# ishine/ASR-Rescoring

Measured on AMD Instinct MI355X. Metric: masked-token BERT forwards/sec (MLM_PLL, N=50, L~32), higher is better.
Workload: dtype fp16x3-split (fp32-accurate: hi/lo fp16 operand split on fp16 MFMA, fp32 accumulate)

## Files before the change

### asr-rescoring_amd/_lib.py

```python
from __future__ import annotations

import ctypes
import os

import numpy as np
import torch

PKG_DIR = os.path.dirname(os.path.abspath(__file__))
LIB_PATH = os.environ.get("RS_LIBRESCORE") or os.path.join(PKG_DIR, "librescore.so")

RS_HEAD_MLM, RS_HEAD_CLS, RS_HEAD_EMB = 1, 2, 4
RS_FUSE = {"norm": 0, "legacy": 1, "am_norm": 2}
KINDS = ["qkv", "oproj", "ffn1", "ffn2", "decoder", "attn", "other"]


class RsBertCfg(ctypes.Structure):
    _fields_ = [("vocab", ctypes.c_int32), ("hidden", ctypes.c_int32), ("layers", ctypes.c_int32),
                ("heads", ctypes.c_int32), ("intermediate", ctypes.c_int32),
                ("max_pos", ctypes.c_int32), ("type_vocab", ctypes.c_int32),
                ("ln_eps", ctypes.c_float), ("mask_id", ctypes.c_int32),
                ("heads_mask", ctypes.c_int32), ("precision", ctypes.c_int32)]


RS_PREC = {"fp16": 0, "fp16x3": 1}
# ... 73 lines not shown
    "rs_trainer_destroy": (None, [P]),
    "rs_bertscore_recall": (ctypes.c_int, [P, P, P, P, I32, P, P, P]),
    "rs_align": (ctypes.c_int, [P, P, P, P, I32, P, P, P, P, P, P, P, I32, P]),
    "rs_fuse_rerank": (ctypes.c_int, [P, P, P, P, I32, I32, P, I32, I32, P, P]),
    "rs_corpus_edits": (ctypes.c_int, [P, P, P, I32, I32, P, P]),
    "rs_ref_edit": (ctypes.c_int, [P, P, P, P, P, I32, P, P]),
    "rs_vocab_load": (P, [ctypes.c_char_p]),
    "rs_vocab_size": (ctypes.c_int, [P]),
    "rs_vocab_free": (None, [P]),
    "rs_vocab_continuation": (ctypes.c_int, [P, P, I64, P]),
    "rs_tokenize_batch": (I64, [P, ctypes.POINTER(ctypes.c_char_p), I32, I32, P, I64, P]),
    "rs_json_write_scores": (ctypes.c_int, [ctypes.c_char_p, I32, ctypes.POINTER(ctypes.c_char_p), P,
                                            ctypes.POINTER(ctypes.c_char_p), P]),
}

CI = ctypes.c_int
_DEBUG_SIGS = {
    "rs_debug_gemm": (CI, [CI, CI, P, P, P, P, CI, CI, CI, P]),
    "rs_debug_attention": (CI, [CI, P, P, P, CI, CI, CI, P, P]),
    "rs_debug_ln": (CI, [CI, CI] + [P] * 9),
    "rs_debug_stamps": (CI, [CI, P]),
    "rs_debug_occupy": (CI, [CI, CI, P, P]),
    "rs_debug_sgemm_cfg": (CI, [CI] * 4 + [P, CI, CI, P, CI, CI, P, CI, CI, P]),
    "rs_debug_sgemm": (CI, [CI] * 3 + [P, CI, CI, P, CI, CI, P, CI, CI, P]),
    "rs_debug_sgemm_pick": (CI, [CI] * 5),
    "rs_debug_gelu": (CI, [P, P, CI, P]),
    "rs_debug_x3s": (CI, [CI, P, P, P, P, P, ctypes.c_float, P, CI, CI, CI, CI, CI, P, P, P, P]),
    "rs_debug_lnres_sizes": (CI, [CI, CI, ctypes.POINTER(I64)]),
    "rs_debug_attention_full": (CI, [P, P, P, CI, CI, CI, CI, CI, P, P]),
    "rs_debug_gemm_epi": (CI, [CI, P, P, CI, CI, CI, P, P]),
    "rs_debug_decoder": (CI, [P, P, P, P, CI, CI, CI, CI, CI, P, P, P, P, P]),
    "rs_debug_decoder_topk": (CI, [P, P, P, P, CI, CI, CI, CI, CI, P, P, P, P, CI, P, P, P, P]),
    "rs_debug_attention_query": (CI, [P, CI, P, P, P, CI, CI, CI, CI, CI, CI, P, P, P, P, P, P, P, P, P]),
    "rs_debug_train_attn": (CI, [CI, P, P, P, CI, CI, CI, P, ctypes.c_uint32, ctypes.c_uint64, ctypes.c_uint32,
                                 ctypes.c_float, P, P, P]),
    "rs_debug_train_embed_ln": (CI, [P, P, P, CI, CI, CI, CI, P, P, P, P, P, ctypes.c_float, CI, ctypes.c_uint32,
                                     ctypes.c_uint64, ctypes.c_uint32, ctypes.c_float, P, P, P, P]),
    "rs_debug_train_bias_res_ln": (CI, [P, P, P, CI, P, P, ctypes.c_float, CI, ctypes.c_uint32, ctypes.c_uint64,
                                        ctypes.c_uint32, ctypes.c_float, P, P, P]),
    "rs_debug_train_ln_bwd": (CI, [P, P, P, P, P, CI, CI, P]),
    "rs_debug_train_pointwise": (CI, [CI, P, P, P, CI, CI, P]),
    "rs_debug_train_colsum": (CI, [CI, P, P, P, CI, CI, P, P, CI, P, CI, P]),
    "rs_debug_train_word_grad": (CI, [P, P, P, P, CI, CI, CI, CI, P, P]),
    "rs_debug_train_pos_grad": (CI, [P, P, CI, CI, CI, CI, P, P]),
    "rs_debug_train_cls_fwd": (CI, [P, P, CI, CI, CI, P, P, P, P]),
    "rs_debug_train_cls_bwd": (CI, [P, P, P, CI, CI, CI, P, P, P, P, P]),
    "rs_debug_train_loss": (CI, [P, P, P, P, P, CI, CI, CI, ctypes.c_float, P, P, P, P]),
    "rs_debug_train_ce": (CI, [P, P, CI, CI, P, P, P]),
    "rs_debug_train_move_rows": (CI, [CI, P, P, CI, CI, CI, P, P]),
    "rs_debug_train_adamw": (CI, [P, P, P, P, I64] + [ctypes.c_float] * 5 + [I64, P]),
    "rs_debug_train_adamw_scaled": (CI, [P, P, P, P, I64] + [ctypes.c_float] * 6 + [I64, P]),
    "rs_debug_train_accum": (CI, [P, P, P, P, CI, I64, ctypes.c_float, P]),
    "rs_debug_train_sumsq": (CI, [P, P, P, CI, I64, P, P]),
    "rs_debug_bertscore_recall": (CI, [P, CI, CI, P, P, CI, P, P, P]),
    "rs_debug_embed_out": (CI, [P, P, P, P, P, P, P, P, CI, CI, CI, CI, CI, P, P]),
    "rs_debug_plan_unique": (CI, [P, P, P, P, CI, CI, CI, P, P]),
    "rs_debug_embed": (CI, [CI, P, P, P, CI, CI, CI, CI, CI, CI, CI, P, P, P, P, P, ctypes.c_float, CI, P, P, P, CI, P]),
    "rs_debug_attention_plan": (CI, [P, CI, P, CI, CI, CI, CI, CI, CI, CI, CI, P, P]),
    "rs_debug_attention_mquery": (CI, [P, CI, P, CI, CI, CI, CI, CI, P, P, P, P, P, P, P, P, P]),
    "rs_debug_gather": (CI, [CI, P, CI, P, P, CI, CI, CI, P, P, P, P]),
    "rs_debug_cls_linear": (CI, [P, CI, CI, P, P, P, P]),
    "rs_debug_segsum": (CI, [P, P, CI, P, P]),
}


class DebugGemmEpi(ctypes.Structure):
# ... 65 lines not shown
```

### asr-rescoring_amd/csrc/common.h

```cpp
#pragma once
#include <hip/hip_runtime.h>
#include <stdint.h>

typedef _Float16 f16;
typedef _Float16 half8 __attribute__((ext_vector_type(8)));
typedef _Float16 half4 __attribute__((ext_vector_type(4)));
typedef float f32x16 __attribute__((ext_vector_type(16)));
typedef float f32x4 __attribute__((ext_vector_type(4)));

#define RS_WAVE 64

enum EpiKind {
    EPI_BIAS_F16 = 0,
    EPI_GELU_F16 = 1,
    EPI_GELU_F32 = 2,
    EPI_RES_F32 = 3,
    EPI_LSE = 4,
    EPI_BIAS_F32 = 5,
    EPI_RESLN_F32 = 6,
    EPI_LNRES_IMG = 7,
    EPI_LSE_TOPK = 8,
};

struct EpiArgs {
// ... 125 lines not shown
}

hipError_t launch_embed_ln(const int* tok, const int* type, SeqMeta sm, int s0, int s1, int row0, int mask_id,
                           int vocab, int type_vocab, const float* word, const float* pos, const float* typetab,
                           const float* g, const float* b, float eps, int H, float* x32,
                           float2* stats, f16* h16, int kx, hipStream_t st);
hipError_t launch_ln_rows(const float* x, int rows, const float* g, const float* b, float eps,
                          int H, float* y32, float2* stats, f16* y16, int kx, hipStream_t st);
hipError_t launch_ln_res_rows(float* x32, const float2* stats, float2* stats_out, const float* pg, const float* pb,
                             const f16* o16, int rows, const float* g, const float* b, float eps, int H,
                             f16* y16, bool write_x, hipStream_t st, const float2* stats1 = nullptr,
                             const float* g1 = nullptr, const float* b1 = nullptr, const f16* o16b = nullptr);
hipError_t launch_ln_res32(float* x32, const float2* stats, float2* stats_out, const float* pg, const float* pb,
                           const float* o32, int rows, const float* g, const float* b, float eps, int H, f16* y16,
                           int kx, hipStream_t st);
hipError_t launch_ln_res_img(f16* h16, const float* o32, int rows, const float* g, const float* b, float eps, int H,
                             hipStream_t st);
hipError_t launch_embed_unique(const int* tok, const int* type, SeqMeta sm, int s0, int s1, int urows, int mask_id,
                               int vocab, int type_vocab, const float* word, const float* pos, const float* typetab,
                               const float* g, const float* b, float eps, int H, f16* h16u, int kx, hipStream_t st);
int bertscore_cols(bool two);
hipError_t launch_bertscore_recall(const f16* emb, int H, const int* hyp_off, const int* utt_off,
                                   const long long* mat_off, const int4* items, int n_items, float* rmat, float* rmat0,
                                   hipStream_t st, bool two = false);
hipError_t launch_embed_out(const float* x32, const float2* stats, const float* g, const float* b,
                            SeqMeta sm, int s0, int s1, int row0, int H, f16* out, hipStream_t st,
                            const f16* himg = nullptr, bool two = false);
hipError_t launch_attention_full(const void* qkv, bool qkv32, SeqMeta sm, int s0, int s1, int row0,
                                 int H, int heads, f16* ctx, int kx, hipStream_t st, bool dedup, int max_len);
hipError_t launch_attention_query(const void* qkv, bool qkv32, const float* x32, const float2* stats,
                                  const float* g, const float* b, SeqMeta sm, int s0, int s1,
                                  int row0, int H, int heads, f16* ctxq, float* resq, int kx,
                                  hipStream_t st, const void* qd = nullptr, const f16* himg = nullptr);
hipError_t launch_gather_query_rows(const f16* src, int ld, SeqMeta sm, int s0, int s1, int row0, f16* dst,
                                   hipStream_t st);
hipError_t launch_gather_labels(const int* tok, SeqMeta sm, int s0, int s1, int* lab, float* label_logit,
                                hipStream_t st);
hipError_t launch_lse_finalize(const float2* part, int n_parts, const float* label_logit,
                               int rows, float* out, hipStream_t st);
hipError_t launch_embed_ln_set(const int* tok, const int* type, SeqMeta sm, QueryMeta qm, int s0, int s1, int mask_id,
                               int vocab, int type_vocab, const float* word, const float* pos, const float* typetab,
                               const float* g, const float* b, float eps, int H, float* x32, float2* stats, f16* h16,
                               int kx, hipStream_t st);
hipError_t launch_attention_mquery(const void* qkv, bool qkv32, const float* x32, const float2* stats, const float* g,
                                   const float* b, SeqMeta sm, QueryMeta qm, int s0, int s1, int H, int heads,
                                   f16* ctxq, float* resq, int kx, hipStream_t st, const void* qd = nullptr,
                                   const f16* himg = nullptr);
hipError_t launch_gather_query_rows_list(const f16* src, int ld, SeqMeta sm, QueryMeta qm, int q0, int n, f16* dst,
                                        hipStream_t st);
hipError_t launch_gather_labels_list(const int* tok, SeqMeta sm, QueryMeta qm, int q0, int n, int* lab,
                                     float* label_logit, hipStream_t st);

struct MlmDecoder {
    const f16* A;
    const f16* W;
    const float* bias;
    int m_valid, vpad, vocab, K;
    const int* tok;
    SeqMeta sm;
    int s0;
    int* lab;
    float2* part;
    float* llog;
    float* out;
    const QueryMeta* qm = nullptr;
};
// ... 52 lines not shown
```

### asr-rescoring_amd/csrc/k_attn.hip

```cpp
#include <type_traits>
#include "common.h"

namespace {

typedef __fp16 fp16x4 __attribute__((__vector_size__(4 * sizeof(__fp16))));

__device__ __forceinline__ half4 tr_read(const f16* p) {
    const fp16x4 v = __builtin_amdgcn_ds_read_tr16_b64_v4f16((__attribute__((address_space(3))) fp16x4*)p);
    return __builtin_bit_cast(half4, v);
}

template <class QT, bool DEDUP>
struct SeqRows {
    const QT* base;
    const QT* mbase;
    int ld, lo, n;
    __device__ __forceinline__ SeqRows(const QT* qkv, const SeqMeta& sm, int s, int rs, int ld_, int hd) : ld(ld_) {
        const int ub = DEDUP ? sm.urow_h[s] : rs;
        lo = DEDUP ? sm.mask_pos[s] : 0;
        n = DEDUP ? sm.mask_end[s] - lo : 0;
        const int um = DEDUP ? sm.urow_m[s] - lo : 0;
        base = qkv + (size_t)ub * ld + hd * 64;
        mbase = qkv + (ptrdiff_t)um * ld + hd * 64;
    }
// ... 582 lines not shown
                float d = 0.f;
#pragma unroll
                for (int c = 0; c < 8; ++c) {
                    float kv[8];
                    load8(kr + c * 8, kv);
#pragma unroll
                    for (int e = 0; e < 8; ++e) d += sq[w][c * 8 + e] * kv[e];
                }
                sc = d;
            }
            const float mn = fmaxf(m, wave_max(sc));
            const float p = (j < T) ? __expf(sc - mn) : 0.f;
            const float alpha = __expf(m - mn);
            l = l * alpha + wave_sum(p);
            acc *= alpha;
            __syncthreads();
            sp[w][lane] = p;
            __syncthreads();
            const int nk = min(64, T - k0);
            for (int jj = 0; jj < nk; ++jj)
                acc += sp[w][jj] * (float)base[(size_t)(k0 + jj) * ld + 2 * H + lane];
            m = mn;
        }
        if (on) {
            put_split(ctxq + (size_t)q_loc * kx * H, h * 64 + lane, H, kx, acc / l);
            const int c = h * 64 + lane;
            const size_t r = (size_t)(rs + qi);
            const float2 hl = himg ? il_parts(himg + r * 2 * H, c) : make_float2(0.f, 0.f);
            resq[(size_t)q_loc * H + c] = himg ? hl.x + hl.y * X3_DOWN : ln_apply(x32[r * H + c], stats[r], lg[c], lb[c]);
        }
    }
}

__global__ void __launch_bounds__(256)
attn_memskel_kernel(const f16* __restrict__ qkv, SeqMeta sm, int H, f16* __restrict__ ctx, int heads_per_block) {
    const int s = blockIdx.x;
    const int T = sm.len[s], rs = sm.row[s];
    const int lane = threadIdx.x & 63, hd = blockIdx.y * heads_per_block + (threadIdx.x >> 6);
    const int ld = 3 * H;
    const f16* base = qkv + (size_t)rs * ld + hd * 64;
    for (int r0 = 0; r0 < T; r0 += 8) {
        const int t = r0 + (lane >> 3), d0 = (lane & 7) * 8;
        if (t < T) {
            const half8 q = *(const half8*)(base + (size_t)t * ld + d0);
            const half8 k = *(const half8*)(base + (size_t)t * ld + H + d0);
            const half8 v = *(const half8*)(base + (size_t)t * ld + 2 * H + d0);
            *(half8*)(ctx + (size_t)(rs + t) * H + hd * 64 + d0) = q + k + v;
        }
    }
}

enum AttnKind {
    ATTN_TR = 0,
    ATTN_MEMSKEL_1 = 3,
    ATTN_MEMSKEL_4 = 4,
    ATTN_16 = 6,
    ATTN_FULL_F32 = 9,
    ATTN_X3_48 = 10,
    ATTN_X3_64 = 11,
};

}

hipError_t launch_attention_full(const void* qkv, bool qkv32, SeqMeta sm, int s0, int s1, int row0,
                                 int H, int heads, f16* ctx, int kx, hipStream_t st, bool dedup, int max_len) {
    if (s1 <= s0) return hipSuccess;
// ... 12 lines not shown
            if (max_len <= 64) hipLaunchKernelGGL(attn16_kernel<D>, grid, block, 0, st, q, sm, s0, row0, H, ctx, kx);
            else hipLaunchKernelGGL(attn_tr_kernel<D>, grid, block, 0, st, q, sm, s0, row0, H, ctx, kx);
        }
    };
    if (dedup) route(std::true_type{});
    else route(std::false_type{});
    return hipGetLastError();
}

hipError_t launch_attention_query(const void* qkv, bool qkv32, const float* x32, const float2* stats,
                                  const float* g, const float* b, SeqMeta sm, int s0, int s1,
                                  int row0, int H, int heads, f16* ctxq, float* resq, int kx,
                                  hipStream_t st, const void* qd, const f16* himg) {
    if (s1 <= s0) return hipSuccess;
    const dim3 grid(s1 - s0, heads);
    if (qkv32)
        hipLaunchKernelGGL(attn_query_kernel<float>, grid, dim3(64), 0, st, (const float*)qkv, (const float*)qd, x32, stats, g, b, sm, s0, row0, H, ctxq, resq, kx, himg);
    else
        hipLaunchKernelGGL(attn_query_kernel<f16>, grid, dim3(64), 0, st, (const f16*)qkv, (const f16*)qd, x32, stats, g, b, sm, s0, row0, H, ctxq, resq, kx, himg);
    return hipGetLastError();
}

hipError_t launch_attention_mquery(const void* qkv, bool qkv32, const float* x32, const float2* stats, const float* g,
                                   const float* b, SeqMeta sm, QueryMeta qm, int s0, int s1, int H, int heads,
                                   f16* ctxq, float* resq, int kx, hipStream_t st, const void* qd, const f16* himg) {
    if (s1 <= s0) return hipSuccess;
    if (H != heads * 64) return hipErrorInvalidValue;
    const dim3 grid(s1 - s0, heads);
    if (qkv32)
        hipLaunchKernelGGL(attn_mquery_kernel<float>, grid, dim3(256), 0, st, (const float*)qkv, (const float*)qd, x32, stats, g, b, sm, qm, s0, H, ctxq, resq, kx, himg);
    else
        hipLaunchKernelGGL(attn_mquery_kernel<f16>, grid, dim3(256), 0, st, (const f16*)qkv, (const f16*)qd, x32, stats, g, b, sm, qm, s0, H, ctxq, resq, kx, himg);
    return hipGetLastError();
}

extern "C" int rs_debug_attention(int kind, const void* qkv, const int* len, const int* row, int n_seq,
                                  int H, int heads, void* ctx, void* stream) {
    SeqMeta sm{};
    sm.len = len;
    sm.row = row;
    const dim3 grid(n_seq, heads), block(64);
    hipStream_t st = (hipStream_t)stream;
    const f16* q16 = (const f16*)qkv;
    const float* q32 = (const float*)qkv;
    f16* c = (f16*)ctx;
    switch (kind) {
        case ATTN_TR: hipLaunchKernelGGL(attn_tr_kernel<false>, grid, block, 0, st, q16, sm, 0, 0, H, c, 1); break;
        case ATTN_16: hipLaunchKernelGGL(attn16_kernel<false>, grid, block, 0, st, q16, sm, 0, 0, H, c, 1); break;
        case ATTN_FULL_F32: hipLaunchKernelGGL(attn_full_kernel<float>, grid, block, 0, st, q32, sm, 0, 0, H, c, 3, 0); break;
        case ATTN_X3_48: hipLaunchKernelGGL((attn16x3v2_kernel<false, 48>), grid, block, 0, st, q32, sm, 0, 0, H, c, 3); break;
        case ATTN_X3_64: hipLaunchKernelGGL((attn16x3v2_kernel<false, 64>), grid, block, 0, st, q32, sm, 0, 0, H, c, 3); break;
        case ATTN_MEMSKEL_1: hipLaunchKernelGGL(attn_memskel_kernel, grid, block, 0, st, q16, sm, H, c, 1); break;
        case ATTN_MEMSKEL_4:
            hipLaunchKernelGGL(attn_memskel_kernel, dim3(n_seq, heads / 4), dim3(256), 0, st, q16, sm, H, c, 4);
            break;
        default: return -1;
    }
    return hipGetLastError() == hipSuccess ? 0 : -2;
}

extern "C" int rs_debug_attention_full(const void* qkv32, const int* len, const int* row, int n_seq, int max_len,
                                       int H, int heads, int kx, void* ctx, void* stream) {
    if (!qkv32 || !len || !row || !ctx || n_seq <= 0 || max_len <= 0 || heads <= 0 || H != heads * 64) return -1;
    if (kx != 2 && kx != 3) return -1;
    SeqMeta sm{};
    sm.len = len;
// ... 46 lines not shown
```

### asr-rescoring_amd/csrc/rs_api.hip

```cpp
#include <map>
#include <string>
#include <vector>
#include <cstring>
#include <cstdio>
#include <cmath>
#include <algorithm>

#include "common.h"
#include "seq_plan.h"
#include "bertscore_plan.h"
#include "host_util.h"

namespace {

thread_local std::string g_err;

int fail(int code, const std::string& msg) {
    g_err = msg;
    return code;
}

struct Layer {
    f16 *wqkv, *wo, *w1, *w2;
    f16 *iqkv = nullptr, *io = nullptr, *i1 = nullptr, *i2 = nullptr;
    float *bqkv, *bo, *b1, *b2, *g1, *be1, *g2, *be2;
};

struct Staging {
    int* p = nullptr;
    size_t cap = 0;
    hipEvent_t done = nullptr;
    hipError_t begin(size_t n) {
        hipError_t e = done ? hipEventSynchronize(done) : hipSuccess;
        if (e == hipSuccess && n > cap) {
            if (p) (void)hipHostFree(p);
            p = nullptr;
            e = hipHostMalloc((void**)&p, std::max<size_t>(n, 1) * 4, hipHostMallocDefault);
            cap = e == hipSuccess ? n : 0;
        }
        return e;
    }
    hipError_t upload(DevBuf& dst, size_t n, hipStream_t st) {
        hipError_t e = dst.ensure(std::max<size_t>(n, 1) * 4);
        if (e == hipSuccess) e = hipMemcpyAsync(dst.p, p, n * 4, hipMemcpyHostToDevice, st);
        if (e == hipSuccess && !done) e = hipEventCreateWithFlags(&done, hipEventDisableTiming);
        return e == hipSuccess ? hipEventRecord(done, st) : e;
    }
    ~Staging() {
        if (p) (void)hipHostFree(p);
        if (done) (void)hipEventDestroy(done);
    }
};

}

struct rs_model {
    rs_bert_cfg cfg{};
    int device = 0;
// ... 270 lines not shown
    ~ProfScope() {
        if (m->prof && a) {
            hipEvent_t b = next_event(m);
            if (b) {
                (void)hipEventRecord(b, st);
                m->recs.push_back({kind, a, b, flops});
            }
        }
    }
};

#define LAUNCH(kind_, call_) do { ProfScope ps_(m, st, (kind_), 0); TRY_HIP(call_); } while (0)
#define LAUNCH_OTHER(call_) LAUNCH(RS_K_OTHER, call_)

enum Mode { MODE_MLM = 0, MODE_CLS = 1, MODE_EMB = 2 };

struct Call {
    int mode;
    const int* d_tok;
    float* out_rows = nullptr;
    const int* d_label = nullptr;
    const int32_t* d_type = nullptr;
    const std::vector<int>* extra = nullptr;
    int** d_extra = nullptr;
    f16* emb_dst = nullptr;
    int topk_k = 0;
    int32_t* topk_id = nullptr;
    float* topk_lp = nullptr;
    const QueryList* ql = nullptr;
};

struct CallOpts {
    bool lastq, dedup, chunk_align;
    int ln_diag;
    bool x3s, imgres, lnfuse, x3_dedup;
    bool oproj_f16, ffn2_f16;
    int lnres_defer;
};

CallOpts call_opts(const rs_model* m) {
    const rs_bert_cfg& cf = m->cfg;
    auto is = [](const char* name, const char* v) { const char* e = getenv(name); return e && !strcmp(e, v); };
    auto num = [](const char* name, int dflt) { const char* e = getenv(name); return e ? atoi(e) : dflt; };
    CallOpts o{};
    o.lastq = !is("RS_LASTQ", "0");
    o.dedup = num("RS_DEDUP", 1) != 0;
    o.chunk_align = !is("RS_CHUNK_ALIGN", "0");
    o.oproj_f16 = m->kx == 1 && !is("RS_OPROJ", "resln");
    o.ffn2_f16 = m->kx == 1 && is("RS_FFN2", "f16");
    const int defer = num("RS_LNRES_DEFER", 2);
    o.lnres_defer = !o.oproj_f16 || o.ffn2_f16 || defer == 0 ? 0 : defer == 2 ? 2 : 1;
    o.ln_diag = num("RS_LNFUSE_DIAG", 0) & 8;
    o.x3s = m->kx == 3 && !is("RS_X3S", "0") && m->x3s_w && cf.hidden % 256 == 0 && cf.intermediate % 256 == 0;
    o.imgres = o.x3s && !is("RS_X3S_IMGRES", "0");
    o.lnfuse = o.imgres && !is("RS_LNFUSE", "0") && cf.hidden % 256 == 0 && cf.hidden <= 1024;
    o.x3_dedup = o.imgres;
    return o;
}

struct ChunkCtx {
    rs_model* m;
    hipStream_t st;
    const Call& call;
    const SeqMeta& sm;
    const Chunk& c;
    const CallOpts& o;
    const QueryMeta& qm;
    const rs_bert_cfg& cf = m->cfg;
    const int H = cf.hidden, F = cf.intermediate, nh = cf.heads, kx = m->kx;
    const float eps = cf.ln_eps;
    const bool q32 = kx == 3;
    const int qkv_epi = q32 ? EPI_BIAS_F32 : EPI_BIAS_F16;
    const int rows = c.rows, ns = c.s1 - c.s0;
    const bool mq = call.ql != nullptr;
    const int nr = mq ? c.nq : ns, r0 = mq ? c.q0 : c.s0;
    const bool dedup = c.urows > 0;
    const int kxf = o.x3s ? 2 : kx;
    float2 *xst = m->xst.as<float2>(), *xst1 = m->xst1.as<float2>();
    float* t32 = m->t32.as<float>();
    f16* h16 = m->h16.as<f16>();
    void* qkv = m->qkv.p;
    f16 *ctx = m->ctx.as<f16>(), *inter = m->inter.as<f16>();
    f16 *ctxq = m->ctxq.as<f16>(), *hq16 = m->hq16.as<f16>(), *interq = m->interq.as<f16>();
    float *resq = m->resq.as<float>(), *tq = m->tq32.as<float>(), *hq32 = m->hq32.as<float>();

    int gemm(int kind, int epi, bool split, const f16* A, const f16* W, int m_valid, int N_pad, int K, EpiArgs ep,
             int n_flop_cols) {
        ep.m_valid = m_valid;
        ProfScope ps(m, st, kind, 2.0 * m_valid * (double)n_flop_cols * (split ? 3.0 * K : K));
// ... 15 lines not shown
    EpiArgs resln_ep(const float* bias, const float* lg, const float* lb) const {
        EpiArgs e = bias_ep(bias, t32, H, t32);
        e.res_stats = xst; e.res_g = lg; e.res_b = lb;
        return e;
    }
    const float* prev_g(int li) const { return li ? m->layers[li - 1].g2 : m->eg; }
    const float* prev_b(int li) const { return li ? m->layers[li - 1].be2 : m->eb; }
    int embed() {
        ProfScope ps(m, st, RS_K_OTHER, 0);
        if (mq && call.ql->masked) {
            TRY_HIP(launch_embed_ln_set(call.d_tok, call.d_type, sm, qm, c.s0, c.s1, cf.mask_id, cf.vocab, cf.type_vocab,
                                       m->word32, m->pos32, m->type32, m->eg, m->eb, eps, H, o.imgres ? nullptr : t32,
                                       o.imgres ? nullptr : xst, h16, kxf, st));
            return RS_OK;
        }
        TRY_HIP(launch_embed_ln(call.d_tok, call.d_type, sm, c.s0, c.s1, 0, cf.mask_id, cf.vocab, cf.type_vocab, m->word32,
                               m->pos32, m->type32, m->eg, m->eb, eps, H, o.imgres ? nullptr : t32,
                               o.imgres ? nullptr : xst, dedup && !o.x3s ? nullptr : h16, kxf, st));
        if (dedup)
            TRY_HIP(launch_embed_unique(call.d_tok, call.d_type, sm, c.s0, c.s1, c.urows, cf.mask_id, cf.vocab,
                                       cf.type_vocab, m->word32, m->pos32, m->type32, m->eg, m->eb, eps, H,
                                       o.x3s ? inter : h16, kxf, st));
        return RS_OK;
    }

    int qkv_proj(int li, bool last, bool uq, bool qrow) {
        const Layer& L = m->layers[li];
        const bool sp = o.x3s;
        const f16* W = sp ? L.iqkv : L.wqkv;
        const int K = sp ? H : kx * H, ldw = sp ? 2 * H : kx * H;
        if (!qrow)
            return gemm(RS_K_QKV, qkv_epi, sp, uq && sp ? inter : h16, W, uq ? c.urows : rows, 3 * H, K,
                        bias_ep(L.bqkv, qkv, 3 * H), last ? 2 * H : 3 * H);
        if (int r = gemm(RS_K_QKV, qkv_epi, sp, h16, W + (size_t)H * ldw, rows, 2 * H, K,
                         bias_ep(L.bqkv + H, (char*)qkv + H * (size_t)(q32 ? 4 : 2), 3 * H), 2 * H)) return r;
        if (mq) LAUNCH_OTHER(launch_gather_query_rows_list(h16, kxf * H, sm, qm, c.q0, c.nq, hq16, st));
        else LAUNCH_OTHER(launch_gather_query_rows(h16, kxf * H, sm, c.s0, c.s1, 0, hq16, st));
        return gemm(RS_K_QKV, qkv_epi, sp, hq16, W, nr, H, K, bias_ep(L.bqkv, tq, H), H);
    }

    int split_block(int kind, const f16* A, const f16* W, int K, const float* bias, const float* pg, const float* pb,
                    const float* g, const float* be) {
        if (o.lnfuse) {
            EpiArgs e = bias_ep(bias, h16, 2 * H);
            e.nlog = H; e.res_g = g; e.res_b = be; e.ln_eps = eps; e.lnx = m->lnx.p;
            e.lncnt = m->lncnt.as<unsigned>(); e.lnerr = m->lnerr.as<unsigned>(); e.diag = o.ln_diag;
            return gemm(kind, EPI_LNRES_IMG, true, A, W, rows, H, K, e, H);
        }
        float* o32 = (float*)qkv;
        if (int r = gemm(kind, EPI_BIAS_F32, true, A, W, rows, H, K, bias_ep(bias, o32, H), H)) return r;
        if (o.imgres) LAUNCH_OTHER(launch_ln_res_img(h16, o32, rows, g, be, eps, H, st));
        else LAUNCH_OTHER(launch_ln_res32(t32, xst, xst, pg, pb, o32, rows, g, be, eps, H, h16, 2, st));
        return RS_OK;
    }
    int layer_split(int li, bool uq) {
        const Layer& L = m->layers[li];
        LAUNCH(RS_K_ATTN, launch_attention_full(qkv, true, sm, c.s0, c.s1, 0, H, nh, ctx, 2, st, uq, c.max_len));
        if (int r = split_block(RS_K_OPROJ, ctx, L.io, H, L.bo, prev_g(li), prev_b(li), L.g1, L.be1)) return r;
        if (int r = gemm(RS_K_FFN1, EPI_GELU_F16, true, h16, L.i1, rows, F, H, gelu_ep(L.b1, inter, 2), F)) return r;
        return split_block(RS_K_FFN2, inter, L.i2, F, L.b2, L.g1, L.be1, L.g2, L.be2);
    }

    int layer_f16(int li, bool uq) {
        const Layer& L = m->layers[li];
        const float *pg = prev_g(li), *pb = prev_b(li);
        LAUNCH(RS_K_ATTN, launch_attention_full(qkv, q32, sm, c.s0, c.s1, 0, H, nh, ctx, kx, st, uq, c.max_len));
        f16* o16 = o.lnres_defer ? (f16*)qkv : inter;
        if (!o.oproj_f16) {
            if (int r = gemm(RS_K_OPROJ, EPI_RESLN_F32, false, ctx, L.wo, rows, H, kx * H, resln_ep(L.bo, pg, pb), H))
                return r;
            LAUNCH_OTHER(launch_ln_rows(t32, rows, L.g1, L.be1, eps, H, nullptr, xst, h16, kx, st));
        } else {
            if (int r = gemm(RS_K_OPROJ, EPI_BIAS_F16, false, ctx, L.wo, rows, H, H, bias_ep(L.bo, o16, H), H)) return r;
            if (o.lnres_defer)
                LAUNCH_OTHER(launch_ln_res_rows(t32, xst, xst1, pg, pb, o16, rows, L.g1, L.be1, eps, H, h16, false, st));
            else
                LAUNCH_OTHER(launch_ln_res_rows(t32, xst, xst, pg, pb, o16, rows, L.g1, L.be1, eps, H, h16, true, st));
        }
        if (int r = gemm(RS_K_FFN1, EPI_GELU_F16, false, h16, L.w1, rows, F, kx * H, gelu_ep(L.b1, inter, kx), F)) return r;
        if (o.lnres_defer == 2) {
            if (int r = gemm(RS_K_FFN2, EPI_BIAS_F16, false, inter, L.w2, rows, H, F, bias_ep(L.b2, ctx, H), H)) return r;
            LAUNCH_OTHER(launch_ln_res_rows(t32, xst, xst, pg, pb, o16, rows, L.g2, L.be2, eps, H, h16, true, st, xst1,
                                            L.g1, L.be1, ctx));
        } else if (o.ffn2_f16) {
            if (int r = gemm(RS_K_FFN2, EPI_BIAS_F16, false, inter, L.w2, rows, H, F, bias_ep(L.b2, ctx, H), H)) return r;
            LAUNCH_OTHER(launch_ln_res_rows(t32, xst, xst, L.g1, L.be1, ctx, rows, L.g2, L.be2, eps, H, h16, true, st));
        } else if (o.lnres_defer == 1) {
            EpiArgs ep = resln_ep(L.b2, L.g1, L.be1);
            ep.res_stats = xst1; ep.res_o16 = o16; ep.res_stats0 = xst; ep.res_g0 = pg; ep.res_b0 = pb;
            if (int r = gemm(RS_K_FFN2, EPI_RESLN_F32, false, inter, L.w2, rows, H, kx * F, ep, H)) return r;
            LAUNCH_OTHER(launch_ln_rows(t32, rows, L.g2, L.be2, eps, H, nullptr, xst, h16, kx, st));
        } else {
            if (int r = gemm(RS_K_FFN2, EPI_RESLN_F32, false, inter, L.w2, rows, H, kx * F, resln_ep(L.b2, L.g1, L.be1), H))
                return r;
            LAUNCH_OTHER(launch_ln_rows(t32, rows, L.g2, L.be2, eps, H, nullptr, xst, h16, kx, st));
        }
        return RS_OK;
    }

    int layer_query(int li, bool qrow) {
        const Layer& L = m->layers[li];
        if (mq)
            LAUNCH(RS_K_ATTN, launch_attention_mquery(qkv, q32, t32, xst, prev_g(li), prev_b(li), sm, qm, c.s0, c.s1, H, nh,
                                                      ctxq, resq, kx, st, qrow ? tq : nullptr, o.imgres ? h16 : nullptr));
        else
            LAUNCH(RS_K_ATTN, launch_attention_query(qkv, q32, t32, xst, prev_g(li), prev_b(li), sm, c.s0, c.s1, 0, H, nh,
                                                     ctxq, resq, kx, st, qrow ? tq : nullptr, o.imgres ? h16 : nullptr));
        if (int r = gemm(RS_K_OPROJ, EPI_RES_F32, false, ctxq, L.wo, nr, H, kx * H, bias_ep(L.bo, tq, H, resq), H))
            return r;
        LAUNCH_OTHER(launch_ln_rows(tq, nr, L.g1, L.be1, eps, H, hq32, nullptr, hq16, kx, st));
        if (int r = gemm(RS_K_FFN1, EPI_GELU_F16, false, hq16, L.w1, nr, F, kx * H, gelu_ep(L.b1, interq, kx), F)) return r;
        if (int r = gemm(RS_K_FFN2, EPI_RES_F32, false, interq, L.w2, nr, H, kx * F, bias_ep(L.b2, tq, H, hq32), H))
            return r;
        LAUNCH_OTHER(launch_ln_rows(tq, nr, L.g2, L.be2, eps, H, hq32, nullptr, hq16, kx, st));
        return RS_OK;
    }

    int head_mlm() {
        if (int r = gemm(RS_K_DECODER, EPI_GELU_F32, false, hq16, m->wt, nr, H, kx * H, bias_ep(m->bt, tq, H), H)) return r;
        LAUNCH_OTHER(launch_ln_rows(tq, nr, m->gt, m->bet, eps, H, hq32, nullptr, hq16, kx, st));
        const MlmDecoder d{hq16, m->wdec, m->bdec, nr, m->vpad, cf.vocab, kx * H, call.d_tok, sm, r0, m->lab.as<int>(),
                           m->part.as<float2>(), m->llog.as<float>(), call.out_rows + r0, mq ? &qm : nullptr};
        if (call.topk_k) {
            const int k = call.topk_k, n_gemm = (ns + TOPK_SUB_ROWS - 1) / TOPK_SUB_ROWS;
            const MlmTopk t{k, m->topk_cand.as<float2>(), call.topk_id + (size_t)c.s0 * k, call.topk_lp + (size_t)c.s0 * k};
            TRY_HIP(launch_mlm_decoder_topk(d, t, st, [&](bool is_gemm, auto&& launch) {
                ProfScope ps(m, st, is_gemm ? RS_K_DECODER : RS_K_OTHER,
                             is_gemm ? 2.0 * ns * (double)cf.vocab * (kx * H) / n_gemm : 0);
                return launch();
            }));
            return RS_OK;
        }
        TRY_HIP(launch_mlm_decoder(d, st, [&](bool is_gemm, auto&& launch) {
            ProfScope ps(m, st, is_gemm ? RS_K_DECODER : RS_K_OTHER, is_gemm ? 2.0 * nr * (double)cf.vocab * (kx * H) : 0);
            return launch();
// ... 333 lines not shown
        auto* bq = need(m, p + "attention.self.query.bias", H, &miss);
        auto* wk = need(m, p + "attention.self.key.weight", H * H, &miss);
        auto* bk = need(m, p + "attention.self.key.bias", H, &miss);
        auto* wv = need(m, p + "attention.self.value.weight", H * H, &miss);
        auto* bv = need(m, p + "attention.self.value.bias", H, &miss);
        auto* wo = need(m, p + "attention.output.dense.weight", H * H, &miss);
        auto* bo = need(m, p + "attention.output.dense.bias", H, &miss);
        auto* g1 = need(m, p + "attention.output.LayerNorm.weight", H, &miss);
        auto* be1 = need(m, p + "attention.output.LayerNorm.bias", H, &miss);
        auto* w1 = need(m, p + "intermediate.dense.weight", F * H, &miss);
        auto* b1 = need(m, p + "intermediate.dense.bias", F, &miss);
        auto* w2 = need(m, p + "output.dense.weight", H * F, &miss);
        auto* b2 = need(m, p + "output.dense.bias", H, &miss);
        auto* g2 = need(m, p + "output.LayerNorm.weight", H, &miss);
        auto* be2 = need(m, p + "output.LayerNorm.bias", H, &miss);
        if (!miss.empty()) return fail(RS_ESTATE, "tensor " + miss);
        std::vector<float> wqkv, bqkv;
        wqkv.reserve(3 * H * H);
        for (auto* w : {wq, wk, wv}) wqkv.insert(wqkv.end(), w->begin(), w->end());
        for (auto* b : {bq, bk, bv}) bqkv.insert(bqkv.end(), b->begin(), b->end());
        Layer& L = m->layers[i];
        UP16(L.wqkv, &wqkv, 3 * H, H);
        UP32(L.bqkv, &bqkv, 3 * H);
        UP16(L.wo, wo, H, H);
        UP32(L.bo, bo, H);
        UP32(L.g1, g1, H);
        UP32(L.be1, be1, H);
        UP16(L.w1, w1, F, H);
        UP32(L.b1, b1, F);
        UP16(L.w2, w2, H, F);
        UP32(L.b2, b2, H);
        UP32(L.g2, g2, H);
        UP32(L.be2, be2, H);
        if (x3s_w) {
            UPIL(L.iqkv, &wqkv, H);
            UPIL(L.io, wo, H);
            UPIL(L.i1, w1, H);
            UPIL(L.i2, w2, F);
        }
    }
#undef UPIL
    m->x3s_w = x3s_w;
    if (c.heads_mask & RS_HEAD_MLM) {
        const std::string p = "cls.predictions.";
        auto* wt = need(m, p + "transform.dense.weight", H * H, &miss);
        auto* bt = need(m, p + "transform.dense.bias", H, &miss);
        auto* gt = need(m, p + "transform.LayerNorm.weight", H, &miss);
        auto* bet = need(m, p + "transform.LayerNorm.bias", H, &miss);
        auto* bd = need(m, p + "bias", V, &miss);
        if (!miss.empty()) return fail(RS_ESTATE, "tensor " + miss);
        auto it = m->host.find(p + "decoder.weight");
        const std::vector<float>* dec = word;
        if (it != m->host.end()) {
            if (it->second.size() != V * H) return fail(RS_EARG, "decoder.weight has wrong size");
            dec = &it->second;
        }
        m->vpad = (int)((V + 127) / 128 * 128);
        UP16(m->wt, wt, H, H);
        UP32(m->bt, bt, H);
        UP32(m->gt, gt, H);
        UP32(m->bet, bet, H);
        UP16(m->wdec, dec, (size_t)m->vpad, H);
        UP32(m->bdec, bd, (size_t)m->vpad);
    }
    if (c.heads_mask & RS_HEAD_CLS) {
        auto* wl = need(m, "linear.weight", H, &miss);
// ... 335 lines not shown
```

Before: 68490.

## Fold K/V projections into query-side attention for the last layer

```diff
diff --git a/asr-rescoring_amd/_lib.py b/asr-rescoring_amd/_lib.py
--- a/asr-rescoring_amd/_lib.py
+++ b/asr-rescoring_amd/_lib.py
@@ -129,6 +129,7 @@
     "rs_debug_decoder": (CI, [P, P, P, P, CI, CI, CI, CI, CI, P, P, P, P, P]),
     "rs_debug_decoder_topk": (CI, [P, P, P, P, CI, CI, CI, CI, CI, P, P, P, P, CI, P, P, P, P]),
     "rs_debug_attention_query": (CI, [P, CI, P, P, P, CI, CI, CI, CI, CI, CI, P, P, P, P, P, P, P, P, P]),
+    "rs_debug_attention_fold": (CI, [P, P, P, P, P, P, P, P, CI, CI, CI, CI, CI, CI, P, ctypes.c_longlong, P, P, P]),
     "rs_debug_train_attn": (CI, [CI, P, P, P, CI, CI, CI, P, ctypes.c_uint32, ctypes.c_uint64, ctypes.c_uint32,
                                  ctypes.c_float, P, P, P]),
     "rs_debug_train_embed_ln": (CI, [P, P, P, CI, CI, CI, CI, P, P, P, P, P, ctypes.c_float, CI, ctypes.c_uint32,
diff --git a/asr-rescoring_amd/csrc/common.h b/asr-rescoring_amd/csrc/common.h
--- a/asr-rescoring_amd/csrc/common.h
+++ b/asr-rescoring_amd/csrc/common.h
@@ -181,6 +181,40 @@
                                   const float* g, const float* b, SeqMeta sm, int s0, int s1,
                                   int row0, int H, int heads, f16* ctxq, float* resq, int kx,
                                   hipStream_t st, const void* qd = nullptr, const f16* himg = nullptr);
+struct AttnFold {
+    const f16* himg;
+    const float *tq, *wkf, *wvt, *bv;
+    SeqMeta sm;
+    int s0, s1, row0, H, heads, kx;
+    void* work;
+    size_t work_bytes;
+    f16* ctxq;
+    float* resq;
+};
+bool attention_fold_ok(int H, int heads);
+hipError_t launch_gather_q32(const float* src, int ld, SeqMeta sm, int s0, int s1, int row0, int H, float* dst,
+                             hipStream_t st);
+hipError_t launch_fold_in(const AttnFold& a, int s0, int n, float* G, hipStream_t st);
+hipError_t launch_fold_query(const AttnFold& a, int s0, int n, const float* G, float* U, hipStream_t st);
+hipError_t launch_fold_out(const AttnFold& a, int s0, int n, const float* U, hipStream_t st);
+template <class Wrap>
+hipError_t launch_attention_fold(const AttnFold& a, hipStream_t st, Wrap&& wrap) {
+    if (a.s1 <= a.s0) return hipSuccess;
+    if (!attention_fold_ok(a.H, a.heads)) return hipErrorInvalidValue;
+    const size_t per = (size_t)a.heads * a.H;
+    const size_t cap = a.work_bytes / (2 * per * sizeof(float));
+    if (cap == 0) return hipErrorInvalidValue;
+    for (int s = a.s0; s < a.s1;) {
+        const int n = (int)(cap < (size_t)(a.s1 - s) ? cap : (size_t)(a.s1 - s));
+        float *G = (float*)a.work, *U = G + (size_t)n * per;
+        const double flops = 2.0 * n * (double)a.H * a.H;
+        if (hipError_t e = wrap(0, flops, [&] { return launch_fold_in(a, s, n, G, st); })) return e;
+        if (hipError_t e = wrap(1, 0.0, [&] { return launch_fold_query(a, s, n, G, U, st); })) return e;
+        if (hipError_t e = wrap(0, flops, [&] { return launch_fold_out(a, s, n, U, st); })) return e;
+        s += n;
+    }
+    return hipSuccess;
+}
 hipError_t launch_gather_query_rows(const f16* src, int ld, SeqMeta sm, int s0, int s1, int row0, f16* dst,
                                    hipStream_t st);
 hipError_t launch_gather_labels(const int* tok, SeqMeta sm, int s0, int s1, int* lab, float* label_logit,
diff --git a/asr-rescoring_amd/csrc/k_attn.hip b/asr-rescoring_amd/csrc/k_attn.hip
--- a/asr-rescoring_amd/csrc/k_attn.hip
+++ b/asr-rescoring_amd/csrc/k_attn.hip
@@ -638,6 +638,163 @@
     }
 }
 
+
+template <bool IMG>
+__global__ void __launch_bounds__(256)
+fold_gemm_kernel(const float* __restrict__ A, int lda, int a_bs, const float* __restrict__ B, int ldb, int b_bs,
+                 int M, int K, float* __restrict__ C, int ldc, int c_bs, const float* __restrict__ bias,
+                 f16* __restrict__ img, int Himg, int kx) {
+    const int lane = threadIdx.x & 63, h = lane >> 5, c = lane & 31;
+    const int m0 = (blockIdx.x * 4 + (threadIdx.x >> 6)) * 32, n0 = blockIdx.y * 64, b = blockIdx.z;
+    if (m0 >= M) return;
+    const float* ap = A + (size_t)b * a_bs + (size_t)min(m0 + c, M - 1) * lda + 16 * h;
+    const float* bp = B + (size_t)b * b_bs + (size_t)(16 * h) * ldb + n0 + c;
+    f32x16 acc[2];
+#pragma unroll
+    for (int j = 0; j < 2; ++j)
+#pragma unroll
+        for (int r = 0; r < 16; ++r) acc[j][r] = 0.f;
+    for (int k0 = 0; k0 < K; k0 += 32) {
+        float fa[16], fb[2][16];
+#pragma unroll
+        for (int q = 0; q < 4; ++q) {
+            const float4 v = *(const float4*)(ap + k0 + 4 * q);
+            fa[4 * q] = v.x; fa[4 * q + 1] = v.y; fa[4 * q + 2] = v.z; fa[4 * q + 3] = v.w;
+        }
+#pragma unroll
+        for (int kk = 0; kk < 16; ++kk) {
+            const float* br = bp + (size_t)(k0 + kk) * ldb;
+            fb[0][kk] = br[0];
+            fb[1][kk] = br[32];
+        }
+#pragma unroll
+        for (int kk = 0; kk < 16; ++kk)
+#pragma unroll
+            for (int j = 0; j < 2; ++j)
+                acc[j] = __builtin_amdgcn_mfma_f32_32x32x2f32(fa[kk], fb[j][kk], acc[j], 0, 0, 0);
+    }
+#pragma unroll
+    for (int j = 0; j < 2; ++j) {
+        const int col = n0 + 32 * j + c;
+#pragma unroll
+        for (int r = 0; r < 16; ++r) {
+            const int row = m0 + (r & 3) + 8 * (r >> 2) + 4 * h;
+            if (row >= M) continue;
+            if constexpr (IMG) put_split(img + (size_t)row * kx * Himg, 64 * b + col, Himg, kx, acc[j][r] + bias[64 * b + col]);
+            else C[(size_t)b * c_bs + (size_t)row * ldc + col] = acc[j][r];
+        }
+    }
+}
+
+typedef float f32x2 __attribute__((ext_vector_type(2)));
+template <int CTRL, int ROWS>
+__device__ __forceinline__ float dpp_add(float v) {
+    return v + __builtin_bit_cast(float, __builtin_amdgcn_update_dpp(0, __builtin_bit_cast(int, v), CTRL, ROWS, 0xF, false));
+}
+__device__ __forceinline__ float wave_sum_dpp(float v) {
+    v = dpp_add<0xB1, 0xF>(v);
+    v = dpp_add<0x4E, 0xF>(v);
+    v = dpp_add<0x124, 0xF>(v);
+    v = dpp_add<0x128, 0xF>(v);
+    v = dpp_add<0x142, 0xA>(v);
+    v = dpp_add<0x143, 0xC>(v);
+    return __builtin_bit_cast(float, __builtin_amdgcn_readlane(__builtin_bit_cast(int, v), 63));
+}
+constexpr int FOLD_R = 24;
+template <int NK>
+__global__ void __launch_bounds__(256 * NK, NK <= 3 ? 2 * NK : NK)
+attn_fold_kernel(const f16* __restrict__ himg, const float* __restrict__ G, float* __restrict__ U,
+                 float* __restrict__ resq, SeqMeta sm, int s0, int row0) {
+    constexpr int H = 256 * NK, NT = 256 * NK, R = FOLD_R;
+    __shared__ __attribute__((aligned(16))) float sx[R][H];
+    const int s = s0 + blockIdx.x, s_loc = blockIdx.x;
+    const int T = sm.len[s], rs = sm.row[s] - row0, qi = sm.query[s];
+    const int tid = threadIdx.x, lane = tid & 63, hd = tid >> 6;
+    const f16* img = himg + (size_t)rs * 2 * H;
+    const size_t gu = ((size_t)s_loc * (4 * NK) + hd) * H + 4 * lane;
+    f32x4 g[NK], u[NK];
+#pragma unroll
+    for (int k = 0; k < NK; ++k) {
+        g[k] = *(const f32x4*)(G + gu + 256 * k);
+        u[k] = f32x4{0.f, 0.f, 0.f, 0.f};
+    }
+    float m = -INFINITY, l = 0.f;
+    for (int t0 = 0; t0 < T; t0 += R) {
+        const int nk = min(R, T - t0);
+        half8 vh[R / 8], vl[R / 8];
+#pragma unroll
+        for (int i = 0; i < R / 8; ++i) {
+            const int un = tid + i * NT, r = un / (H / 8), c8 = (un % (H / 8)) * 8;
+            vh[i] = vl[i] = half8{0, 0, 0, 0, 0, 0, 0, 0};
+            if (r < nk) {
+                const f16* p = img + (size_t)(t0 + r) * 2 * H + il_hi(c8);
+                vh[i] = *(const half8*)p;
+                vl[i] = *(const half8*)(p + 32);
+            }
+        }
+        __syncthreads();
+#pragma unroll
+        for (int i = 0; i < R / 8; ++i) {
+            const int un = tid + i * NT, r = un / (H / 8), c8 = (un % (H / 8)) * 8;
+            float x[8];
+#pragma unroll
+            for (int e = 0; e < 8; ++e) x[e] = (float)vh[i][e] + (float)vl[i][e] * X3_DOWN;
+            *(float4*)&sx[r][c8] = make_float4(x[0], x[1], x[2], x[3]);
+            *(float4*)&sx[r][c8 + 4] = make_float4(x[4], x[5], x[6], x[7]);
+        }
+        __syncthreads();
+        float sc = -INFINITY;
+        for (int r0 = 0; r0 < nk; r0 += 4) {
+            float d[4];
+#pragma unroll
+            for (int j = 0; j < 4; ++j) {
+                f32x2 a = {0.f, 0.f};
+#pragma unroll
+                for (int k = 0; k < NK; ++k) {
+                    const f32x4 x = *(const f32x4*)&sx[r0 + j][256 * k + 4 * lane];
+                    a = __builtin_elementwise_fma(g[k].xy, x.xy, a);
+                    a = __builtin_elementwise_fma(g[k].zw, x.zw, a);
+                }
+                d[j] = a.x + a.y;
+            }
+#pragma unroll
+            for (int j = 0; j < 4; ++j) {
+                const float t = wave_sum_dpp(d[j]);
+                if (lane == r0 + j) sc = t;
+            }
+        }
+        if (lane >= nk) sc = -INFINITY;
+        const float mn = fmaxf(m, wave_max(sc));
+        const float p = lane < nk ? __expf(sc - mn) : 0.f;
+        const float alpha = __expf(m - mn);
+        l = l * alpha + wave_sum(p);
+#pragma unroll
+        for (int k = 0; k < NK; ++k) u[k] *= alpha;
+        for (int r0 = 0; r0 < nk; r0 += 4) {
+#pragma unroll
+            for (int j = 0; j < 4; ++j) {
+                const float pr = __builtin_bit_cast(float, __builtin_amdgcn_readlane(__builtin_bit_cast(int, p), r0 + j));
+                const f32x2 pp = {pr, pr};
+#pragma unroll
+                for (int k = 0; k < NK; ++k) {
+                    const f32x4 x = *(const f32x4*)&sx[r0 + j][256 * k + 4 * lane];
+                    u[k].xy = __builtin_elementwise_fma(pp, x.xy, u[k].xy);
+                    u[k].zw = __builtin_elementwise_fma(pp, x.zw, u[k].zw);
+                }
+            }
+        }
+        m = mn;
+    }
+#pragma unroll
+    for (int k = 0; k < NK; ++k)
+        *(f32x4*)(U + gu + 256 * k) = f32x4{u[k].x / l, u[k].y / l, u[k].z / l, u[k].w / l};
+    {
+        const int c = hd * 64 + lane;
+        const float2 hl = il_parts(img + (size_t)qi * 2 * H, c);
+        resq[(size_t)s_loc * H + c] = hl.x + hl.y * X3_DOWN;
+    }
+}
+
 __global__ void __launch_bounds__(256)
 attn_memskel_kernel(const f16* __restrict__ qkv, SeqMeta sm, int H, f16* __restrict__ ctx, int heads_per_block) {
     const int s = blockIdx.x;
@@ -716,6 +873,70 @@
     else
         hipLaunchKernelGGL(attn_mquery_kernel<f16>, grid, dim3(256), 0, st, (const f16*)qkv, (const f16*)qd, x32, stats, g, b, sm, qm, s0, H, ctxq, resq, kx, himg);
     return hipGetLastError();
+}
+
+namespace {
+__global__ void __launch_bounds__(64)
+gather_q32_kernel(const float* __restrict__ src, int ld, SeqMeta sm, int s0, int row0, int H, float* __restrict__ dst) {
+    const int s = s0 + blockIdx.x;
+    const size_t r = (size_t)(sm.row[s] - row0 + sm.query[s]);
+    const float4* a = (const float4*)(src + r * ld);
+    float4* o = (float4*)(dst + (size_t)blockIdx.x * H);
+    for (int i = threadIdx.x; i < H / 4; i += 64) o[i] = a[i];
+}
+}
+
+hipError_t launch_gather_q32(const float* src, int ld, SeqMeta sm, int s0, int s1, int row0, int H, float* dst,
+                             hipStream_t st) {
+    if (s1 <= s0) return hipSuccess;
+    if (H % 4 || ld % 4) return hipErrorInvalidValue;
+    hipLaunchKernelGGL(gather_q32_kernel, dim3(s1 - s0), dim3(64), 0, st, src, ld, sm, s0, row0, H, dst);
+    return hipGetLastError();
+}
+
+bool attention_fold_ok(int H, int heads) { return H == heads * 64 && H % 256 == 0 && H <= 1024; }
+
+hipError_t launch_fold_in(const AttnFold& a, int s0, int n, float* G, hipStream_t st) {
+    const int H = a.H;
+    hipLaunchKernelGGL(fold_gemm_kernel<false>, dim3((n + 127) / 128, H / 64, a.heads), dim3(256), 0, st,
+                       a.tq + (size_t)(s0 - a.s0) * H, H, 64, a.wkf, H, 64 * H, n, 64, G, a.heads * H, H, nullptr,
+                       nullptr, 0, 0);
+    return hipGetLastError();
+}
+
+hipError_t launch_fold_query(const AttnFold& a, int s0, int n, const float* G, float* U, hipStream_t st) {
+    float* resq = a.resq + (size_t)(s0 - a.s0) * a.H;
+    switch (a.H / 256) {
+        case 1: hipLaunchKernelGGL(attn_fold_kernel<1>, dim3(n), dim3(256), 0, st, a.himg, G, U, resq, a.sm, s0, a.row0); break;
+        case 2: hipLaunchKernelGGL(attn_fold_kernel<2>, dim3(n), dim3(512), 0, st, a.himg, G, U, resq, a.sm, s0, a.row0); break;
+        case 3: hipLaunchKernelGGL(attn_fold_kernel<3>, dim3(n), dim3(768), 0, st, a.himg, G, U, resq, a.sm, s0, a.row0); break;
+        case 4: hipLaunchKernelGGL(attn_fold_kernel<4>, dim3(n), dim3(1024), 0, st, a.himg, G, U, resq, a.sm, s0, a.row0); break;
+        default: return hipErrorInvalidValue;
+    }
+    return hipGetLastError();
+}
+
+hipError_t launch_fold_out(const AttnFold& a, int s0, int n, const float* U, hipStream_t st) {
+    const int H = a.H;
+    hipLaunchKernelGGL(fold_gemm_kernel<true>, dim3((n + 127) / 128, 1, a.heads), dim3(256), 0, st, U, a.heads * H, H,
+                       a.wvt, H, 64, n, H, nullptr, 0, 0, a.bv, a.ctxq + (size_t)(s0 - a.s0) * a.kx * H, H, a.kx);
+    return hipGetLastError();
+}
+
+extern "C" int rs_debug_attention_fold(const void* himg, const float* tq, const float* wkf, const float* wvt,
+                                       const float* bv, const int* len, const int* row, const int* query, int s0,
+                                       int s1, int row0, int H, int heads, int kx, void* work, long long work_bytes,
+                                       void* ctxq, float* resq, void* stream) {
+    if (!himg || !tq || !wkf || !wvt || !bv || !len || !row || !query || !work || !ctxq || !resq) return -1;
+    if (s0 < 0 || s1 <= s0 || work_bytes <= 0 || !attention_fold_ok(H, heads) || (kx != 1 && kx != 3)) return -1;
+    AttnFold a{};
+    a.himg = (const f16*)himg; a.tq = tq; a.wkf = wkf; a.wvt = wvt; a.bv = bv;
+    a.sm.len = len; a.sm.row = row; a.sm.query = query;
+    a.s0 = s0; a.s1 = s1; a.row0 = row0; a.H = H; a.heads = heads; a.kx = kx;
+    a.work = work; a.work_bytes = (size_t)work_bytes; a.ctxq = (f16*)ctxq; a.resq = resq;
+    hipStream_t st = (hipStream_t)stream;
+    const hipError_t e = launch_attention_fold(a, st, [](int, double, auto&& launch) { return launch(); });
+    return e == hipSuccess ? 0 : -2;
 }
 
 extern "C" int rs_debug_attention(int kind, const void* qkv, const int* len, const int* row, int n_seq,
diff --git a/asr-rescoring_amd/csrc/rs_api.hip b/asr-rescoring_amd/csrc/rs_api.hip
--- a/asr-rescoring_amd/csrc/rs_api.hip
+++ b/asr-rescoring_amd/csrc/rs_api.hip
@@ -24,6 +24,7 @@
     f16 *wqkv, *wo, *w1, *w2;
     f16 *iqkv = nullptr, *io = nullptr, *i1 = nullptr, *i2 = nullptr;
     float *bqkv, *bo, *b1, *b2, *g1, *be1, *g2, *be2;
+    float *wkf = nullptr, *wvt = nullptr;
 };
 
 struct Staging {
@@ -360,6 +361,7 @@
 
 struct CallOpts {
     bool lastq, dedup, chunk_align;
+    bool lastfold;
     int ln_diag;
     bool x3s, imgres, lnfuse, x3_dedup;
     bool oproj_f16, ffn2_f16;
@@ -383,6 +385,8 @@
     o.imgres = o.x3s && !is("RS_X3S_IMGRES", "0");
     o.lnfuse = o.imgres && !is("RS_LNFUSE", "0") && cf.hidden % 256 == 0 && cf.hidden <= 1024;
     o.x3_dedup = o.imgres;
+    o.lastfold = o.imgres && !is("RS_LASTFOLD", "0") && attention_fold_ok(cf.hidden, cf.heads) &&
+                 !m->layers.empty() && m->layers.back().wkf != nullptr;
     return o;
 }
 
@@ -464,8 +468,10 @@
         if (!qrow)
             return gemm(RS_K_QKV, qkv_epi, sp, uq && sp ? inter : h16, W, uq ? c.urows : rows, 3 * H, K,
                         bias_ep(L.bqkv, qkv, 3 * H), last ? 2 * H : 3 * H);
-        if (int r = gemm(RS_K_QKV, qkv_epi, sp, h16, W + (size_t)H * ldw, rows, 2 * H, K,
-                         bias_ep(L.bqkv + H, (char*)qkv + H * (size_t)(q32 ? 4 : 2), 3 * H), 2 * H)) return r;
+        if (!fold()) {
+            if (int r = gemm(RS_K_QKV, qkv_epi, sp, h16, W + (size_t)H * ldw, rows, 2 * H, K,
+                             bias_ep(L.bqkv + H, (char*)qkv + H * (size_t)(q32 ? 4 : 2), 3 * H), 2 * H)) return r;
+        }
         if (mq) LAUNCH_OTHER(launch_gather_query_rows_list(h16, kxf * H, sm, qm, c.q0, c.nq, hq16, st));
         else LAUNCH_OTHER(launch_gather_query_rows(h16, kxf * H, sm, c.s0, c.s1, 0, hq16, st));
         return gemm(RS_K_QKV, qkv_epi, sp, hq16, W, nr, H, K, bias_ep(L.bqkv, tq, H), H);
@@ -530,9 +536,25 @@
         return RS_OK;
     }
 
+    bool fold() const { return o.lastfold && !mq; }
+    int attention_fold(const Layer& L) {
+        AttnFold a{};
+        a.himg = h16; a.tq = tq; a.wkf = L.wkf; a.wvt = L.wvt; a.bv = L.bqkv + 2 * H;
+        a.sm = sm; a.s0 = c.s0; a.s1 = c.s1; a.row0 = 0; a.H = H; a.heads = nh; a.kx = kx;
+        a.work = qkv; a.work_bytes = m->qkv.bytes; a.ctxq = ctxq; a.resq = resq;
+        TRY_HIP(launch_attention_fold(a, st, [&](int kind, double flops, auto&& launch) {
+            ProfScope ps(m, st, kind == 0 ? RS_K_QKV : RS_K_ATTN, flops);
+            return launch();
+        }));
+        return RS_OK;
+    }
+
     int layer_query(int li, bool qrow) {
         const Layer& L = m->layers[li];
-        if (mq)
+        if (fold()) {
+            if (!qrow) LAUNCH_OTHER(launch_gather_q32((const float*)qkv, 3 * H, sm, c.s0, c.s1, 0, H, tq, st));
+            if (int r = attention_fold(L)) return r;
+        } else if (mq)
             LAUNCH(RS_K_ATTN, launch_attention_mquery(qkv, q32, t32, xst, prev_g(li), prev_b(li), sm, qm, c.s0, c.s1, H, nh,
                                                       ctxq, resq, kx, st, qrow ? tq : nullptr, o.imgres ? h16 : nullptr));
         else
@@ -932,6 +954,16 @@
         UP32(L.b2, b2, H);
         UP32(L.g2, g2, H);
         UP32(L.be2, be2, H);
+        if (x3s_w && i == c.layers - 1 && attention_fold_ok((int)H, c.heads)) {
+            std::vector<float> wkf(H * H), wvt(H * H);
+            for (size_t r = 0; r < H; ++r)
+                for (size_t j = 0; j < H; ++j) {
+                    wkf[r * H + j] = (*wk)[r * H + j] * 0.125f;
+                    wvt[j * H + r] = (*wv)[r * H + j];
+                }
+            UP32(L.wkf, &wkf, H * H);
+            UP32(L.wvt, &wvt, H * H);
+        }
         if (x3s_w) {
             UPIL(L.iqkv, &wqkv, H);
             UPIL(L.io, wo, H);
```

After: 69190, median of 6. 1.01x the previous value.
